# Twinklebear/tray_rust

Hardware: NVIDIA H100
Metric: Mrays/s (primary+secondary) (higher is better)
Workload: dtype f32

## Files before the change

### tray_rust_b200/csrc/trb_api.cu

```cuda
#include <chrono>
#include <dlfcn.h>
#include <nccl.h>
#include <cstdio>
#include <cstdlib>
#include <memory>
#include <thread>
#include <tuple>
#include <cub/device/device_radix_sort.cuh>
#include "trb_host.h"
#include "trb_kernels.cuh"
#include "trb_bvh_build.cuh"
#include "trb_denoise.cuh"

using namespace trbh;

namespace {

thread_local std::string g_error;
unsigned long long g_launches = 0;
trb_status fail(trb_status s, const std::string& msg) { g_error = msg; return s; }

#define CU(call)                                                                                                   \
    do {                                                                                                           \
        cudaError_t e_ = (call);                                                                                   \
// ... 119 lines not shown
        q.q[2 * k + 1] = make_float4(in[node].bmax[0], in[node].bmax[1], in[node].bmax[2], 0.f);
    };
    for (size_t qi = 0; qi < order.size(); ++qi) {
        const uint32_t p = order[qi];
        trb::DQuad& q = out[qi];
        uint32_t axes[2] = {0, 0};
        int h = 0;
        for (uint32_t c : {p + 1, in[p].a}) {
            bool split = false;
            if (!is_leaf(c)) { const uint32_t g0 = c + 1, g1 = in[c].a; split = inside(g0, c) && inside(g1, c); }
            if (split) { slot(q, 2 * h, c + 1, false); slot(q, 2 * h + 1, in[c].a, false); axes[h] = in[c].b & 3u; }
            else { slot(q, 2 * h, c, false); slot(q, 2 * h + 1, 0, true); }
            ++h;
        }
        q.q[1].w = bits_f((in[p].b & 3u) | axes[0] << 2 | axes[1] << 4);
    }
    root_ref = trb::REF_INTERIOR | quad_of[0];
    return ok;
}

}

namespace {
struct Tuning {
    int refill = 8;
    unsigned trace_grid = 0;
    uint32_t sched = 6;
    int quads = 0;
    int exact_box = 0;
    int wide_leaf = 0;
    int pipe = 36;
    int film_v2 = 1;
    int sort = 0;
    int sort_bits = 5;
    int sort_min_round = 1;
    int shade_anim_occ = 4;
    int frame_device = 1;
    int anim_table = 2;
    int shade_split = -1;
    int shade_sort = 1;
    int shade_kind = 1;
    uint64_t pass_paths = 1ull << 24;
    int build_device = 1;
    long long tlas_min = -1;
    int frame_time = 0;
    int tlas_small = 8;
};
constexpr uint32_t kTlasLevelMin = 256;
int env_int(const char* name, int dflt) { const char* v = getenv(name); return v ? (int)strtol(v, nullptr, 0) : dflt; }
void tuning_from_env(Tuning& t) {
    t.refill = env_int("TRB_REFILL", t.refill); t.trace_grid = (unsigned)env_int("TRB_TRACE_GRID", (int)t.trace_grid);
    t.sched = (uint32_t)env_int("TRB_TRACE_SCHED", (int)t.sched); t.quads = env_int("TRB_TRACE_QUADS", t.quads); t.pipe = env_int("TRB_TRACE_PIPE", t.pipe);
    t.wide_leaf = env_int("TRB_TRACE_WIDE_LEAF", t.wide_leaf);
    t.film_v2 = env_int("TRB_FILM_V2", t.film_v2); t.sort = env_int("TRB_SORT", t.sort); t.sort_bits = env_int("TRB_SORT_BITS", t.sort_bits);
    t.sort_min_round = env_int("TRB_SORT_MIN_ROUND", t.sort_min_round); t.shade_split = env_int("TRB_SHADE_SPLIT", t.shade_split); t.anim_table = env_int("TRB_ANIM_TABLE", t.anim_table); t.frame_device = env_int("TRB_FRAME_DEVICE", t.frame_device);
    if (getenv("TRB_PASS_PATHS")) t.pass_paths = strtoull(getenv("TRB_PASS_PATHS"), nullptr, 0);
    t.build_device = env_int("TRB_BUILD_DEVICE", t.build_device);
    t.tlas_min = env_int("TRB_FRAME_TLAS_MIN", (int)t.tlas_min); t.frame_time = env_int("TRB_FRAME_TIME", t.frame_time);
    t.tlas_small = std::max(4, env_int("TRB_FRAME_TLAS_SMALL", t.tlas_small));
}

}

struct BlockList {
    uint32_t key[5];
    std::vector<uint32_t> host;
    uint2* dev = nullptr;
};

struct trb_scene {
    int device = 0;
    int sm_count = 0;
    Tuning tune;
    trb_film film{};
    trb_integrator integrator{};
    std::vector<trb_camera> cameras;
// ... 322 lines not shown
    }
    s->wf_capacity = cap;
    return TRB_OK;
}

void launch_anim_table(trb_scene* s, trb::WfState& wf, size_t n_paths, bool adapt, cudaStream_t st) {
    if (!(s->ds.has_anim && wf.xf_tab && s->tune.anim_table)) { wf.xf_tab = nullptr; return; }
    const size_t items = n_paths * wf.n_anim;
    const uint32_t nu = s->ds.n_uniq_splines;
    if (s->tune.anim_table >= 2 && nu > 0 && nu <= 256) {
        const uint32_t per_iter = std::max(1u, std::min(32u, 128u / nu));
        const size_t smem = (size_t)per_iter * nu * 32 * sizeof(float);
        const unsigned grid = (unsigned)std::min<size_t>((n_paths + per_iter - 1) / per_iter, (size_t)s->sm_count * 16);
        if (adapt) trb::k_wf_anim_table2<true><<<grid, 128, smem, st>>>(s->ds, wf, per_iter);
        else trb::k_wf_anim_table2<<<grid, 128, smem, st>>>(s->ds, wf, per_iter);
    } else {
        const unsigned grid = (unsigned)std::min<size_t>((items + 127) / 128, (size_t)s->sm_count * 16);
        if (adapt) trb::k_wf_anim_table<true><<<grid, 128, 0, st>>>(s->ds, wf);
        else trb::k_wf_anim_table<<<grid, 128, 0, st>>>(s->ds, wf);
    }
    g_launches++;
}

void launch_query_trace(trb_scene* s, const trb::RenderParams& rp, const trb::WfState& wf, uint32_t tflags, bool stats, const uint32_t* q_sorted,
                        cudaStream_t st) {
    const Tuning& tu = s->tune;
    const bool anim = s->ds.has_anim != 0;
    const unsigned resident = stats ? 4u : (anim ? 8u : 9u);
    const unsigned tgrid = (unsigned)s->sm_count * (tu.trace_grid ? tu.trace_grid : 2u * resident);
    const uint32_t sched = std::max(1u, tu.sched);
    if (s->wide_leaf) {
        if (anim) {
            if (stats) trb::k_wf_trace<true, 4, 16, true, true, false, 225><<<tgrid, 128, 0, st>>>(s->ds, rp, wf, 0, tflags, tu.refill, sched, q_sorted);
            else trb::k_wf_trace<false, 8, 12, true, true, false, 225><<<tgrid, 128, 0, st>>>(s->ds, rp, wf, 0, tflags, tu.refill, sched, q_sorted);
        } else if (stats) trb::k_wf_trace<true, 4, 16, false, true, false, 225><<<tgrid, 128, 0, st>>>(s->ds, rp, wf, 0, tflags, tu.refill, sched, q_sorted);
        else trb::k_wf_trace<false, 9, 12, false, true, false, 225><<<tgrid, 128, 0, st>>>(s->ds, rp, wf, 0, tflags, tu.refill, sched, q_sorted);
    } else if (anim) {
        if (stats) trb::k_wf_trace<true, 4, 16, true, true, false, 97><<<tgrid, 128, 0, st>>>(s->ds, rp, wf, 0, tflags, tu.refill, sched, q_sorted);
        else trb::k_wf_trace<false, 8, 12, true, true, false, 97><<<tgrid, 128, 0, st>>>(s->ds, rp, wf, 0, tflags, tu.refill, sched, q_sorted);
    } else if (stats) trb::k_wf_trace<true, 4, 16, false, true, false, 97><<<tgrid, 128, 0, st>>>(s->ds, rp, wf, 0, tflags, tu.refill, sched, q_sorted);
    else trb::k_wf_trace<false, 9, 12, false, true, false, 97><<<tgrid, 128, 0, st>>>(s->ds, rp, wf, 0, tflags, tu.refill, sched, q_sorted);
}

template <int MODE>
void launch_shade(trb_scene* s, const trb::RenderParams& rp, const trb::WfState& wf, uint32_t round, cudaStream_t st) {
    const Tuning& tu = s->tune;
    const bool anim = s->ds.has_anim != 0;
    const unsigned shade_grid = (unsigned)s->sm_count * 4;
    const bool split_auto = s->mixed_materials || (tu.shade_sort && tu.shade_kind && s->material_kinds == (1u << TRB_MAT_MATTE));
    if (tu.shade_split > 0 || (tu.shade_split < 0 && split_auto)) {
        const uint32_t all = 0xffu, own = (tu.shade_sort && tu.shade_kind) ? (s->material_kinds & (1u << TRB_MAT_MATTE)) : 0u;
        const uint32_t rest = tu.shade_sort ? (s->material_kinds & ~own) : all;
        if (anim) {
            trb::k_wf_shade_a<MODE, true, 3><<<shade_grid, 128, 0, st>>>(s->ds, rp, wf, round);
            if (own) trb::k_wf_shade_b<true, 4, TRB_MAT_MATTE><<<shade_grid, 128, 0, st>>>(s->ds, rp, wf, round, own);
            if (rest) trb::k_wf_shade_b<true, 3><<<shade_grid, 128, 0, st>>>(s->ds, rp, wf, round, rest);
            if (own) trb::k_wf_shade_c<MODE, true, 6, TRB_MAT_MATTE><<<(unsigned)s->sm_count * 6, 128, 0, st>>>(s->ds, rp, wf, round, own);
            if (rest) trb::k_wf_shade_c<MODE, true, 4><<<shade_grid, 128, 0, st>>>(s->ds, rp, wf, round, rest);
        } else {
            const unsigned ga = (unsigned)s->sm_count * 6, gb = (unsigned)s->sm_count * 5, gc = (unsigned)s->sm_count * 6;
            trb::k_wf_shade_a<MODE, false, 6><<<ga, 128, 0, st>>>(s->ds, rp, wf, round);
            if (own) trb::k_wf_shade_b<false, 5, TRB_MAT_MATTE><<<gb, 128, 0, st>>>(s->ds, rp, wf, round, own);
            if (rest) trb::k_wf_shade_b<false, 5><<<gb, 128, 0, st>>>(s->ds, rp, wf, round, rest);
            if (own) trb::k_wf_shade_c<MODE, false, 6, TRB_MAT_MATTE><<<gc, 128, 0, st>>>(s->ds, rp, wf, round, own);
// ... 2 lines not shown
        g_launches += 4;
        return;
    }
    if (anim) {
        if constexpr (MODE == 1) trb::k_wf_shade<1, true, 3><<<shade_grid, 128, 0, st>>>(s->ds, rp, wf, round);
        else if constexpr (MODE == 2) trb::k_wf_shade<2, true, 4><<<shade_grid, 128, 0, st>>>(s->ds, rp, wf, round);
        else if (tu.shade_anim_occ >= 4) trb::k_wf_shade<0, true, 4><<<shade_grid, 128, 0, st>>>(s->ds, rp, wf, round);
        else trb::k_wf_shade<0, true, 3><<<shade_grid, 128, 0, st>>>(s->ds, rp, wf, round);
    } else trb::k_wf_shade<MODE, false, 4><<<shade_grid, 128, 0, st>>>(s->ds, rp, wf, round);
    g_launches += 2;
}

trb_status wavefront_rounds(trb_scene* s, const trb::RenderParams& rp, const trb::WfState& wf, uint32_t flags, int mode, cudaStream_t st,
                            const AovRequest* aov = nullptr) {
    const Tuning& tu = s->tune;
    const bool stats = (flags & TRB_RENDER_STATS) != 0, anim = s->ds.has_anim != 0;
    const uint32_t rounds = s->integrator.max_depth + 2;
    const int refill = tu.refill;
    const unsigned resident = (flags & TRB_RENDER_STATS) ? 4u : (tu.pipe == 0 || tu.pipe == 1 || tu.pipe == 33 ? 7u : (tu.pipe == 34 || tu.pipe == 35 || s->ds.has_anim ? 8u : 9u));
    const unsigned tgrid = (unsigned)s->sm_count * (tu.trace_grid ? tu.trace_grid : 2u * resident);
    const uint32_t sched = tu.sched;
    const bool quads = tu.quads != 0;
    const uint32_t tflags = flags | (tu.exact_box ? trb::WF_TRACE_FORCE_EXACT_BOX : 0u);
    if (s->wide_leaf && (sched == 0 || quads || tu.pipe == 0 || tu.pipe == 1 || (tu.pipe >= 33 && tu.pipe <= 35) || tu.pipe == 37))
        return fail(TRB_UNSUPPORTED, "trace.quads, trace.sched 0 and the experimental trace.pipe variants do not read wide mesh leaves (trace.wide_leaf)");
    if (quads && s->quads_dropped) return fail(TRB_UNSUPPORTED, "trace.quads reads DQuad records, which a mesh updated by trb_scene_update_mesh does not have");
    for (uint32_t round = 0; round < rounds; ++round) {
        const uint32_t* q_sorted = nullptr;
        if (tu.sort && (int)round >= tu.sort_min_round) {
            const uint32_t bits = (uint32_t)std::min(trb::WF_SORT_MAX_BITS, std::max(1, tu.sort_bits));
            const unsigned sgrid = (unsigned)s->sm_count * 8;
            trb::k_wf_sort_count<<<sgrid, 256, 0, st>>>(wf, round, bits, tu.sort == 2 ? 1u : 0u);
            trb::k_wf_sort_scan<<<1, 1024, 0, st>>>(wf, 3u * (8u << (3u * bits)));
            trb::k_wf_sort_scatter<<<sgrid, 256, 0, st>>>(wf, round);
            g_launches += 3;
            q_sorted = wf.q_sorted;
        }
        std::pair<cudaEvent_t, cudaEvent_t> ev{nullptr, nullptr};
        if (flags & TRB_RENDER_TIME_TRACE) {
            if (!s->event_pool.empty()) { ev = s->event_pool.back(); s->event_pool.pop_back(); }
            else { CU(cudaEventCreate(&ev.first)); CU(cudaEventCreate(&ev.second)); }
            CU(cudaEventRecord(ev.first, st));
        }
#define TRB_TRACE_LAUNCH(ST, MB, SS, AN, PH, QD, PIPE) trb::k_wf_trace<ST, MB, SS, AN, PH, QD, PIPE><<<tgrid, 128, 0, st>>>(s->ds, rp, wf, round, tflags, refill, sched, q_sorted)
        const bool v2 = tu.pipe != 0;
        if (mode == 2 && round == 0) launch_query_trace(s, rp, wf, tflags, stats, q_sorted, st);
        else if (s->wide_leaf) {
            if (anim) { if (stats) TRB_TRACE_LAUNCH(true, 4, 16, true, true, false, 161); else TRB_TRACE_LAUNCH(false, 8, 12, true, true, false, 161); }
            else if (stats) TRB_TRACE_LAUNCH(true, 4, 16, false, true, false, 161);
            else TRB_TRACE_LAUNCH(false, 9, 12, false, true, false, 161);
        } else if (anim) {
            if (stats) { if (v2) TRB_TRACE_LAUNCH(true, 4, 16, true, true, false, 33); else TRB_TRACE_LAUNCH(true, 4, 16, true, true, false, 0); }
            else if (!v2) TRB_TRACE_LAUNCH(false, 7, 16, true, true, false, 0);
            else if (tu.pipe == 33) TRB_TRACE_LAUNCH(false, 7, 16, true, true, false, 33);
            else if (tu.pipe == 37) TRB_TRACE_LAUNCH(false, 9, 12, true, true, false, 33);
            else TRB_TRACE_LAUNCH(false, 8, 12, true, true, false, 33);
        } else if (stats) {
            if (sched == 0) TRB_TRACE_LAUNCH(true, 4, 16, false, false, false, 0);
            else if (v2) TRB_TRACE_LAUNCH(true, 4, 16, false, true, false, 33); else TRB_TRACE_LAUNCH(true, 4, 16, false, true, false, 0);
        } else if (sched == 0) TRB_TRACE_LAUNCH(false, 7, 16, false, false, false, 0);
        else if (quads) TRB_TRACE_LAUNCH(false, 7, 16, false, true, true, 0);
        else switch (tu.pipe) {
            case 0: TRB_TRACE_LAUNCH(false, 7, 16, false, true, false, 0); break;
            case 1: TRB_TRACE_LAUNCH(false, 7, 16, false, true, false, 1); break;
            case 33: TRB_TRACE_LAUNCH(false, 7, 16, false, true, false, 33); break;
            case 34: TRB_TRACE_LAUNCH(false, 8, 16, false, true, false, 33); break;
            case 35: TRB_TRACE_LAUNCH(false, 8, 12, false, true, false, 33); break;
            case 37: TRB_TRACE_LAUNCH(false, 9, 8, false, true, false, 33); break;
            default: TRB_TRACE_LAUNCH(false, 9, 12, false, true, false, 33); break;
        }
#undef TRB_TRACE_LAUNCH
        if (ev.first) { CU(cudaEventRecord(ev.second, st)); s->trace_events.push_back(ev); }
        if (aov && round == 0) {
            const unsigned agrid = (unsigned)std::min<size_t>((wf.n_paths + 127) / 128, (size_t)s->sm_count * 16);
            float4* lo = mode == 1 ? reinterpret_cast<float4*>(aov->samples) : s->d_aov;
            float4* hi = mode == 1 ? lo + 1 : s->d_aov + s->aov_capacity;
            const uint32_t step = mode == 1 ? 2u : 1u;
            if (anim) trb::k_wf_aov<true><<<agrid, 128, 0, st>>>(s->ds, wf, lo, hi, step);
            else trb::k_wf_aov<false><<<agrid, 128, 0, st>>>(s->ds, wf, lo, hi, step);
            g_launches++;
        }
        if (mode == 0) launch_shade<0>(s, rp, wf, round, st);
        else if (mode == 1) launch_shade<1>(s, rp, wf, round, st);
        else launch_shade<2>(s, rp, wf, round, st);
    }
    CU(cudaGetLastError());
    return TRB_OK;
}

trb_status launch_wavefront(trb_scene* s, const trb::RenderParams& rp, uint32_t flags, int mode, cudaStream_t st, const AovRequest* aov = nullptr) {
    const size_t n_paths = (size_t)rp.n_blocks * 64 * rp.sample_count;
    if (n_paths > s->wf_capacity || n_paths >= (1ull << 30)) return fail(TRB_INVALID_ARG, "pass larger than the wavefront state");
    const Tuning& tu = s->tune;
// ... 1375 lines not shown
uint32_t trb_abi_version(void) { return TRB_ABI_VERSION; }
unsigned long long trb_launch_count(void) { return g_launches; }

trb_status trb_scene_set_option(trb_scene* s, const char* name, long long value) {
    if (!s || !name) return fail(TRB_INVALID_ARG, "null argument");
    Tuning& t = s->tune;
    const std::string k(name);
    if (k == "trace.refill") t.refill = (int)value;
    else if (k == "trace.occupancy" || k == "trace.smem_stack") {}
    else if (k == "trace.grid") t.trace_grid = (unsigned)std::max<long long>(0, value);
    else if (k == "trace.sched") t.sched = (uint32_t)value;
    else if (k == "trace.quads" || k == "frame.device") {
        int& field = k == "trace.quads" ? t.quads : t.frame_device;
        const bool changed = (field != 0) != (value != 0);
        field = (int)value;
        if (changed && s->frame_set) return trb_scene_update_frame(s, s->last_frame, s->last_start, s->last_end);
    }
    else if (k == "frame.tlas_min") {
        const bool changed = t.tlas_min != value;
        t.tlas_min = value;
        if (changed && s->frame_set) return trb_scene_update_frame(s, s->last_frame, s->last_start, s->last_end);
    }
    else if (k == "trace.pipe") t.pipe = (int)value;
    else if (k == "trace.exact_box") t.exact_box = (int)value;
    else if (k == "trace.wide_leaf") {
        t.wide_leaf = (int)value;
        const bool wide = s->needs_wide || value != 0;
        if (wide != s->wide_leaf) { CU(cudaSetDevice(s->device)); return upload_mesh_nodes(s, wide); }
    }
    else if (k == "film.v2") t.film_v2 = (int)value;
    else if (k == "sort.mode") t.sort = (int)value;
    else if (k == "sort.bits") t.sort_bits = (int)std::min<long long>(6, std::max<long long>(1, value));
    else if (k == "sort.min_round") t.sort_min_round = (int)value;
    else if (k == "shade.split") t.shade_split = (int)value;
    else if (k == "shade.sort") t.shade_sort = (int)value;
    else if (k == "shade.kind") t.shade_kind = (int)value;
    else if (k == "anim.table") t.anim_table = (int)value;
    else if (k == "shade.anim_occupancy") t.shade_anim_occ = (int)value;
    else if (k == "pass.paths") { if (value < 64) return fail(TRB_INVALID_ARG, "pass.paths must be >= 64"); t.pass_paths = (uint64_t)value; }
    else return fail(TRB_INVALID_ARG, "unknown option: " + k);
    return TRB_OK;
}

trb_status trb_scene_check_error(trb_scene* s) {
    if (!s) return fail(TRB_INVALID_ARG, "null scene");
    CU(cudaSetDevice(s->device));
// ... 2183 lines not shown
```

### tray_rust_b200/csrc/trb_kernels.cuh

```cuda
#pragma once
#include "trb_device.h"
#include "trb_detmath.cuh"
#include "trb_anim.h"
#include "trb_adaptive.h"
#include "../../include/trb.h"

namespace trb {

struct f3 { float x, y, z; };
TRB_HD __forceinline__ f3 mk(float x, float y, float z) { f3 r; r.x = x; r.y = y; r.z = z; return r; }
__device__ __forceinline__ f3 splat(float v) { return mk(v, v, v); }
__device__ __forceinline__ f3 operator+(f3 a, f3 b) { return mk(a.x + b.x, a.y + b.y, a.z + b.z); }
__device__ __forceinline__ f3 operator-(f3 a, f3 b) { return mk(a.x - b.x, a.y - b.y, a.z - b.z); }
__device__ __forceinline__ f3 operator*(f3 a, f3 b) { return mk(a.x * b.x, a.y * b.y, a.z * b.z); }
__device__ __forceinline__ float ieee_div(float a, float b) { return a / b; }
__device__ __forceinline__ float ieee_sqrt(float a) { return sqrtf(a); }
__device__ __forceinline__ f3 operator/(f3 a, f3 b) { return mk(ieee_div(a.x, b.x), ieee_div(a.y, b.y), ieee_div(a.z, b.z)); }
__device__ __forceinline__ f3 operator*(f3 a, float s) { return mk(a.x * s, a.y * s, a.z * s); }
__device__ __forceinline__ f3 operator*(float s, f3 a) { return mk(s * a.x, s * a.y, s * a.z); }
__device__ __forceinline__ f3 operator/(f3 a, float s) { return mk(ieee_div(a.x, s), ieee_div(a.y, s), ieee_div(a.z, s)); }
__device__ __forceinline__ f3 operator-(f3 a) { return mk(-a.x, -a.y, -a.z); }
__device__ __forceinline__ float dot3(f3 a, f3 b) { return a.x * b.x + a.y * b.y + a.z * b.z; }
__device__ __forceinline__ f3 cross3(f3 a, f3 b) { return mk(a.y * b.z - a.z * b.y, a.z * b.x - a.x * b.z, a.x * b.y - a.y * b.x); }
__device__ __forceinline__ float len2(f3 a) { return a.x * a.x + a.y * a.y + a.z * a.z; }
// ... 322 lines not shown
                const float p0 = __ldg(&in.p0), p1 = __ldg(&in.p1);
                float tt = t.tmax;
                bool h;
                if (shape == TRB_SHAPE_SPHERE) h = sphere_t(p0, lo_, ld_, t.tmin, tt);
                else if (shape == TRB_SHAPE_DISK) h = disk_t(p0, p1, lo_, ld_, t.tmin, tt);
                else h = rect_t(p0, p1, lo_, ld_, t.tmin, tt);
                if (h) {
                    t.tmax = tt;
                    t.h_inst = ii; t.h_prim = 0; t.h_b1 = 0.0f; t.h_b2 = 0.0f;
                    t.found = true;
                    if (t.any_hit) t.sp = 0;
                }
            }
        }
        if (!enter) next = trace_pop(t, stack);
    }
    t.cur = next;
}

constexpr uint32_t ST_POP = 0xfffffffcu;
constexpr uint32_t WF_TRACE_FORCE_EXACT_BOX = 0x40000000u;
constexpr int WF_BURST = 3;
__device__ __forceinline__ bool trace_is_node(uint32_t cur) { return (cur & REF_TAG) == REF_INTERIOR || cur == ST_POP; }
template <bool STATS, bool QUADS, class Stack>
__device__ __forceinline__ void step_nodes(TraceState& t, const Stack& stack, Cnt& cnt, int* err) {
    uint32_t cur = t.cur;
    if (QUADS && cur != ST_POP && t.quad) {
        const float4* __restrict__ rec = reinterpret_cast<const DQuad*>(t.pairs)[cur].q;
        float4 q0, q1, q2, q3, q4, q5, q6, q7;
        ldg256(rec, q0, q1); ldg256(rec + 2, q2, q3); ldg256(rec + 4, q4, q5); ldg256(rec + 6, q6, q7);
        QuadOut qo;
        quad_visit(q0, q1, q2, q3, q4, q5, q6, q7, t.o, t.inv, (t.neg & 1u) != 0, (t.neg & 2u) != 0, (t.neg & 4u) != 0, t.tmin, t.tmax, qo);
        cur = qo.next == QUAD_EMPTY ? ST_POP : qo.next;
        if (qo.p2) {
            if (t.sp >= STACK_DEPTH - 6) { *err = 1; t.sp = 0; cur = ST_DONE; }
            else {
                if (qo.p0) stack.put(t.sp++, qo.e0);
                if (qo.p1) stack.put(t.sp++, qo.e1);
                stack.put(t.sp++, qo.e2);
            }
        } else if (qo.p0 || qo.p1) {
            if (t.sp >= STACK_DEPTH - 6) { *err = 1; t.sp = 0; cur = ST_DONE; }
            else {
                if (qo.p0) stack.put(t.sp++, qo.e0);
                if (qo.p1) stack.put(t.sp++, qo.e1);
            }
// ... 42 lines not shown
    return (h & 4u) ? (u * 2.0f - 1.0f) * 30.0f : (u * 2.0f - 1.0f);
}
__global__ void k_selftest_box(uint32_t n, uint32_t seed, unsigned long long* out) {
    const uint32_t i = blockIdx.x * blockDim.x + threadIdx.x;
    if (i >= n) return;
    uint32_t h = rng_absorb(rng_seed(seed), i);
    float v[14];
    for (int k = 0; k < 14; ++k) { h = mix32(h + 0x9e3779b9u); v[k] = selftest_value(h); }
    const float4 lo = make_float4(fminf(v[0], v[3]), fminf(v[1], v[4]), fminf(v[2], v[5]), 0.0f), hi = make_float4(fmaxf(v[0], v[3]), fmaxf(v[1], v[4]), fmaxf(v[2], v[5]), 0.0f);
    f3 o = mk(v[6], v[7], v[8]);
    if ((h & 0x30u) == 0) o.x = lo.x;
    if ((h & 0xc0u) == 0) o.y = hi.y;
    const f3 d = mk(v[9], v[10], v[11]);
    const f3 inv = mk(1.0f / d.x, 1.0f / d.y, 1.0f / d.z);
    const float tmin = (h & 0x100u) ? 0.0f : 0.001f, tmax = (h & 0x200u) ? finf() : fabsf(v[12]) * 40.0f;
    const bool nx = d.x < 0.0f, ny = d.y < 0.0f, nz = d.z < 0.0f;
    if (!(finite3(o) && finite3(d) && finite3(inv))) { atomicAdd(&out[3], 1ull); return; }
    float ta = 0.0f, tb = 0.0f;
    const bool a = box_hit(lo, hi, o, inv, nx, ny, nz, tmin, tmax, ta), b = box_hit_finite(lo, hi, o, inv, nx, ny, nz, tmin, tmax, tb);
    atomicAdd(&out[0], 1ull);
    if (a) atomicAdd(&out[1], 1ull);
    if (a != b || (a && !(ta == tb))) atomicAdd(&out[2], 1ull);
}
template <bool STATS, bool FAST, class Stack>
__device__ __forceinline__ void step_nodes2(TraceState& t, const Stack& stack, Cnt& cnt, int* err) {
    uint32_t cur = t.cur;
    if (cur != ST_POP) {
        const DPair* __restrict__ rec = t.pairs + cur;
        float4 l_lo, l_hi, r_lo, r_hi;
        ldg256(&rec->l_lo, l_lo, l_hi);
        ldg256(&rec->r_lo, r_lo, r_hi);
        if (STATS) cnt.node += 2;
        const uint32_t axis = __float_as_uint(r_lo.w);
        const bool neg = ((t.neg >> axis) & 1u) != 0;
        const uint32_t ref_l = __float_as_uint(l_lo.w), ref_r = __float_as_uint(l_hi.w);
        const bool nx = (t.neg & 1u) != 0, ny = (t.neg & 2u) != 0, nz = (t.neg & 4u) != 0;
        float tl, tr;
        bool hl, hr;
        if (FAST && !t.exact_box) {
            hl = box_hit_finite(l_lo, l_hi, t.o, t.inv, nx, ny, nz, t.tmin, t.tmax, tl);
            hr = box_hit_finite(r_lo, r_hi, t.o, t.inv, nx, ny, nz, t.tmin, t.tmax, tr);
        } else {
            hl = box_hit(l_lo, l_hi, t.o, t.inv, nx, ny, nz, t.tmin, t.tmax, tl);
            hr = box_hit(r_lo, r_hi, t.o, t.inv, nx, ny, nz, t.tmin, t.tmax, tr);
        }
        const bool both = hl && hr;
        cur = both ? (neg ? ref_r : ref_l) : (hl ? ref_l : (hr ? ref_r : ST_POP));
        if (both) {
            if (t.sp >= STACK_DEPTH - 6) { *err = 1; t.sp = 0; cur = ST_DONE; }
            else stack.put(t.sp++, ((unsigned long long)__float_as_uint(neg ? tl : tr) << 32) | (neg ? ref_l : ref_r));
        }
    }
#pragma unroll
    for (int k = 0; k < 2; ++k) {
// ... 23 lines not shown
        float4 v0, q0, q1, qpad;
        ldg256(&tri->v0, v0, q0);
        ldg256(&tri->e1, q1, qpad);
        if (WIDE) next = __float_as_uint(q0.w) == TRI_LEAF_END ? ST_POP : cur + 1;
        if (STATS) cnt.tri++;
        const f3 e0 = mk(q0.x, q0.y, q0.z), e1 = mk(q1.x, q1.y, q1.z);
        const f3 s0 = cross3(t.d, e1);
        const float dd = dot3(s0, e0);
        const float div = 1.0f / dd;
        const f3 dv = t.o - mk(v0.x, v0.y, v0.z);
        const float b1 = dot3(dv, s0) * div;
        const f3 s1 = cross3(dv, e0);
        const float b2 = dot3(t.d, s1) * div;
        const float tt = dot3(e1, s1) * div;
        const bool ok = dd != 0.0f && !(b1 < 0.0f || b1 > 1.0f) && !(b2 < 0.0f || b1 + b2 > 1.0f) && !(tt < t.tmin || tt > t.tmax);
        if (ok) {
            t.tmax = tt;
            accept_hit<HOME>(t, home, t.level_inst, __float_as_uint(v0.w), b1, b2);
            if (t.any_hit) { t.sp = 0; next = ST_DONE; }
        }
    }
    t.cur = next;
}
template <bool STATS, bool ANIM, bool HOME = false, class Stack>
__device__ __forceinline__ void step_other(const DScene& sc, TraceState& t, const Stack& stack, Cnt& cnt, const RayHome* home = nullptr) {
    uint32_t cur = t.cur;
    uint32_t next = ST_POP;
    bool inst_now = false;
    if ((cur & REF_TAG) == REF_LEAF) {
        const uint32_t a = cur & 0x01ffffffu, n = (cur >> 25) & 31u;
        if (HOME) {
            for (uint32_t k = a + n; k-- > a + 1;) stack.put(t.sp++, ST_INSTANCE | k);
            cur = ST_INSTANCE | a; inst_now = n != 0;
        } else
            for (uint32_t k = a + n; k-- > a;) stack.put(t.sp++, ST_INSTANCE | k);
    } else if (cur == ST_ROOT) {
        const DBvh* bvh = t.bvh;
        if (HOME) bvh = t.level_inst == TRB_MISS ? sc.tlas : &sc.meshes[__ldg(&sc.instances[t.level_inst].mesh)].bvh;
        const float4 lo = __ldg(&bvh->root_lo), hi = __ldg(&bvh->root_hi);
        if (STATS) cnt.node++;
        float te;
        if (box_hit(lo, hi, t.o, t.inv, (t.neg & 1u) != 0, (t.neg & 2u) != 0, (t.neg & 4u) != 0, t.tmin, t.tmax, te)) next = __float_as_uint(t.quad ? hi.w : lo.w);
    } else if (cur == ST_RETURN) {
        if (HOME) {
            const float4 o4 = __ldcs(home->org), d4 = __ldcs(home->dir);
            t.o = mk(o4.x, o4.y, o4.z); t.d = mk(d4.x, d4.y, d4.z);
            t.inv = mk(1.0f / t.d.x, 1.0f / t.d.y, 1.0f / t.d.z);
        } else { t.o = t.wo; t.d = t.wd; t.inv = t.winv; }
        t.neg = neg_mask(t.d);
        trace_level(t, sc.tlas, sc.tlas_pairs, sc.tlas_quads);
        t.level_inst = TRB_MISS;
    } else inst_now = true;
    if (inst_now) {
        const uint32_t ii = __ldg(&sc.tlas_order[cur & ~REF_TAG]);
        const DInstance& in = sc.instances[ii];
        if (STATS) cnt.inst++;
        const uint32_t kind = __ldg(&in.kind), shape = __ldg(&in.shape);
        if (kind != TRB_INST_EMITTER_POINT) {
            float m[16];
            instance_inv<ANIM>(sc, in, t.time, m, t.xf_row);
            const f3 lo_ = xf_point(m, HOME ? t.o : t.wo), ld_ = xf_vector(m, HOME ? t.d : t.wd);
            if (shape == TRB_SHAPE_MESH) {
                const DMesh& me = sc.meshes[__ldg(&in.mesh)];
                const f3 inv_ = mk(1.0f / ld_.x, 1.0f / ld_.y, 1.0f / ld_.z);
                const uint32_t neg_ = neg_mask(ld_);
                bool enter = true;
                next = ST_ROOT;
                if (HOME) {
                    const float4 lo = __ldg(&me.bvh.root_lo), hi = __ldg(&me.bvh.root_hi);
                    if (STATS) cnt.node++;
                    float te;
                    enter = box_hit(lo, hi, lo_, inv_, (neg_ & 1u) != 0, (neg_ & 2u) != 0, (neg_ & 4u) != 0, t.tmin, t.tmax, te);
                    next = enter ? __float_as_uint(lo.w) : ST_POP;
                }
                if (enter) {
                    t.o = lo_; t.d = ld_; t.inv = inv_; t.neg = neg_;
                    trace_level(t, &me.bvh, me.bvh.pairs, me.bvh.quads);
                    t.tris = me.tris; t.level_inst = ii;
                    stack.put(t.sp++, ST_RETURN);
                }
            } else {
                const float p0 = __ldg(&in.p0), p1 = __ldg(&in.p1);
                float tt = t.tmax;
                bool h;
                if (shape == TRB_SHAPE_SPHERE) h = sphere_t(p0, lo_, ld_, t.tmin, tt);
                else if (shape == TRB_SHAPE_DISK) h = disk_t(p0, p1, lo_, ld_, t.tmin, tt);
                else h = rect_t(p0, p1, lo_, ld_, t.tmin, tt);
                if (h) {
                    t.tmax = tt;
                    accept_hit<HOME>(t, home, ii, 0u, 0.0f, 0.0f);
                    if (t.any_hit) { t.sp = 0; next = ST_DONE; }
                }
            }
        }
    }
    t.cur = next;
// ... 1206 lines not shown
        const PixelStreams ps = pixel_streams(rp.seed, id.pixel);
        float sx, sy, tm;
        sample_position(rp, ps, id, sx, sy, tm);
        Ray ray;
        const float time = camera_ray<ANIM>(sc, sx, sy, tm, ray);
        wf.org[p] = make_float4(ray.o.x, ray.o.y, ray.o.z, __uint_as_float(0u));
        wf.cont[p] = make_float4(ray.d.x, ray.d.y, ray.d.z, finf());
        wf.thr[p] = make_float4(1.0f, 1.0f, 1.0f, time);
        wf.illum[p] = make_float4(0.0f, 0.0f, 0.0f, 0.0f);
        wf.q_cont[p] = p;
    }
    if (blockIdx.x == 0 && threadIdx.x == 0) {
        wf.counters[WF_N_ACTIVE] = n; wf.counters[WF_N_CONT] = n;
        if (rp.stats) { atomicAdd(&rp.stats->camera_samples, (unsigned long long)n); }
    }
    if (wf.bounds && blockIdx.x == 0 && threadIdx.x < 64) {
        uint32_t* b = wf.bounds + threadIdx.x * 8;
        b[0] = b[1] = b[2] = b[3] = 0xffffffffu; b[4] = b[5] = b[6] = b[7] = 0u;
    }
}

template <bool STATS, int MINB, int SMEM_STACK, bool ANIM, bool PHASED, bool QUADS, int PIPE = 0>
__global__ void __launch_bounds__(128, MINB) k_wf_trace(const __grid_constant__ DScene sc, const __grid_constant__ RenderParams rp, const __grid_constant__ WfState wf,
                                                         uint32_t round, uint32_t flags, int WF_REFILL_IDLE, uint32_t sched, const uint32_t* __restrict__ q_sorted) {
    constexpr bool HOME = PHASED && (PIPE & 32) != 0;
    constexpr bool QUERY = (PIPE & 64) != 0;
    constexpr bool WIDE = (PIPE & 128) != 0;
    uint32_t* cnt_r = wf.counters + round * WF_CNT;
    const uint32_t n_cont = cnt_r[WF_N_CONT], n_shadow = cnt_r[WF_N_SHADOW], n_mis = cnt_r[WF_N_MIS];
    const uint32_t total = n_cont + n_shadow + n_mis;
    const bool shadow_any = (flags & 4u) == 0;
    const int lane = threadIdx.x & 31;
    const unsigned lt_mask = (1u << lane) - 1u;
    Cnt cnt = {0, 0, 0};
    TraceState t;
    __shared__ unsigned long long s_stack[SMEM_STACK * 128];
    unsigned long long stack_lo[STACK_DEPTH - SMEM_STACK];
    const HybridStack<SMEM_STACK> stack{s_stack + threadIdx.x, stack_lo};
    t.cur = ST_DONE;
    bool have = false, exhausted = false;
    uint32_t p = 0;
    int type = 0;
    for (;;) {
        if (HOME && have && t.cur == ST_DONE) {
            if (type == 0) {
                __stcs(&wf.cont[p].w, t.tmax);
                if (!t.found) __stcs(&wf.hit[p], make_uint4(TRB_MISS, 0u, 0u, 0u));
            } else if (type == 1) __stcs(&wf.shadow[p].w, __uint_as_float(t.found ? 1u : 0u));
            else {
                __stcs(&wf.mis[p].w, t.tmax);
                if (!t.found) __stcs(&wf.a[p].w, __uint_as_float(TRB_MISS));
            }
            have = false;
        } else if (have && t.cur == ST_DONE) {
            if (type == 0) {
                __stcs(&wf.cont[p], make_float4(t.wd.x, t.wd.y, t.wd.z, t.tmax));
                __stcs(&wf.hit[p], make_uint4(t.found ? t.h_inst : TRB_MISS, t.h_prim, __float_as_uint(t.h_b1), __float_as_uint(t.h_b2)));
            } else if (type == 1) {
                __stcs(&wf.shadow[p], make_float4(t.wd.x, t.wd.y, t.wd.z, __uint_as_float(t.found ? 1u : 0u)));
            } else {
                __stcs(&wf.mis[p], make_float4(t.wd.x, t.wd.y, t.wd.z, t.tmax));
// ... 9 lines not shown
            uint32_t base = 0;
            if (lane == leader) base = atomicAdd(&cnt_r[WF_TRACE_HEAD], (uint32_t)__popc(idle));
            base = __shfl_sync(0xffffffffu, base, leader);
            if (base >= total) exhausted = true;
            else if (!have) {
                const uint32_t i = base + __popc(idle & lt_mask);
                if (i < total) {
                    if (q_sorted) { const uint32_t e = __ldg(&q_sorted[i]); type = (int)(e >> 30); p = e & WF_PATH_MASK; }
                    else if (i < n_cont) { type = 0; p = wf.q_cont[i]; }
                    else if (i < n_cont + n_shadow) { type = 1; p = wf.q_shadow[i - n_cont]; }
                    else { type = 2; p = wf.q_mis[i - n_cont - n_shadow]; }
                    const float4 o4 = __ldcs(&wf.org[p]);
                    const float4 d4 = __ldcs(type == 0 ? &wf.cont[p] : (type == 1 ? &wf.shadow[p] : &wf.mis[p]));
                    Ray ray; ray.o = mk(o4.x, o4.y, o4.z); ray.d = mk(d4.x, d4.y, d4.z);
                    ray.tmin = QUERY ? o4.w : ((type == 0 && round == 0) ? 0.0f : 0.001f);
                    ray.tmax = QUERY ? d4.w : (type == 1 ? 0.999f : finf());
                    trace_init(sc, t, ray, type == 1 && shadow_any, ANIM ? __ldg(&wf.thr[p].w) : 0.0f, QUADS && PHASED, (flags & WF_TRACE_FORCE_EXACT_BOX) != 0);
                    t.xf_row = wf_xf_row<ANIM>(wf, p);
                    if (PHASED) { stack.put(0, (unsigned long long)ST_DONE); t.sp = 1; }
                    if (HOME) {
                        const float4 lo = __ldg(&sc.tlas->root_lo), hi = __ldg(&sc.tlas->root_hi);
                        if (STATS) cnt.node++;
                        float te;
                        t.cur = box_hit(lo, hi, t.o, t.inv, (t.neg & 1u) != 0, (t.neg & 2u) != 0, (t.neg & 4u) != 0, t.tmin, t.tmax, te) ? __float_as_uint(lo.w) : ST_POP;
                    }
                    have = true;
                }
            }
        }
        const unsigned busy0 = __ballot_sync(0xffffffffu, have);
        if (busy0 == 0) { if (exhausted) break; else continue; }
        if (PHASED) {
            const int thr_o = (int)(sched & 255u);
            for (;;) {
#pragma unroll
                for (int k = 0; k < WF_BURST; ++k)
                    if (trace_is_node(t.cur)) {
                        if (PIPE != 0 && !QUADS) step_nodes2<STATS, (PIPE & 1) != 0>(t, stack, cnt, rp.error_flag);
                        else step_nodes<STATS, QUADS>(t, stack, cnt, rp.error_flag);
                    }
                const bool is_a = trace_is_node(t.cur), is_o = !is_a && t.cur != ST_DONE;
                const unsigned m_a = __ballot_sync(0xffffffffu, is_a), m_o = __ballot_sync(0xffffffffu, is_o);
                if ((m_a | m_o) == 0) break;
                if (!exhausted && 32 - __popc(m_a | m_o) >= WF_REFILL_IDLE) break;
                if (m_o != 0 && (m_a == 0 || __popc(m_o) >= thr_o)) {
                    if (is_o) {
                        const RayHome home{&wf.org[p], type == 0 ? &wf.cont[p] : (type == 1 ? &wf.shadow[p] : &wf.mis[p]), &wf.hit[p], &wf.a[p].w, type};
                        if ((t.cur & REF_TAG) == REF_LEAF && t.level_inst != TRB_MISS) step_triangle<STATS, HOME, WIDE>(t, cnt, &home);
                        else step_other<STATS, ANIM, HOME>(sc, t, stack, cnt, &home);
                    }
                }
            }
        } else {
            for (;;) {
                if (have && t.cur != ST_DONE) trace_step<STATS, ANIM, WIDE>(sc, t, stack, cnt, rp.error_flag);
                const unsigned running = __ballot_sync(0xffffffffu, have && t.cur != ST_DONE);
                if (running == 0) break;
                if (!exhausted && 32 - __popc(running) >= WF_REFILL_IDLE) break;
            }
        }
    }
    if (rp.stats) {
        if (STATS) {
            unsigned long long v[3] = {cnt.node, cnt.tri, cnt.inst};
            for (int k = 0; k < 3; ++k) {
                unsigned long long x = v[k];
                for (int o = 16; o > 0; o >>= 1) x += __shfl_xor_sync(0xffffffffu, x, o);
                if (lane == 0 && x) atomicAdd(&rp.stats->node_tests + k, x);
            }
        }
        if (blockIdx.x == 0 && threadIdx.x == 0) {
            atomicAdd(round == 0 ? &rp.stats->rays_primary : &rp.stats->rays_continuation, (unsigned long long)n_cont);
// ... 1136 lines not shown
```

Measured before the change: 779.5.

## Add optional shared-memory BVH top-node cache and raise refill threshold

```diff
diff --git a/tray_rust_b200/csrc/trb_api.cu b/tray_rust_b200/csrc/trb_api.cu
--- a/tray_rust_b200/csrc/trb_api.cu
+++ b/tray_rust_b200/csrc/trb_api.cu
@@ -165,14 +165,16 @@
 }
 
 namespace {
+constexpr uint32_t NODE_CACHE_DEFAULT = 0, NODE_CACHE_MAX = 480;
 struct Tuning {
-    int refill = 8;
+    int refill = 16;
     unsigned trace_grid = 0;
     uint32_t sched = 6;
     int quads = 0;
     int exact_box = 0;
     int wide_leaf = 0;
     int pipe = 36;
+    uint32_t node_cache = NODE_CACHE_DEFAULT;
     int film_v2 = 1;
     int sort = 0;
     int sort_bits = 5;
@@ -195,6 +197,7 @@
     t.refill = env_int("TRB_REFILL", t.refill); t.trace_grid = (unsigned)env_int("TRB_TRACE_GRID", (int)t.trace_grid);
     t.sched = (uint32_t)env_int("TRB_TRACE_SCHED", (int)t.sched); t.quads = env_int("TRB_TRACE_QUADS", t.quads); t.pipe = env_int("TRB_TRACE_PIPE", t.pipe);
     t.wide_leaf = env_int("TRB_TRACE_WIDE_LEAF", t.wide_leaf);
+    t.node_cache = (uint32_t)std::min<int>((int)NODE_CACHE_MAX, std::max(0, env_int("TRB_TRACE_NODE_CACHE", (int)t.node_cache)));
     t.film_v2 = env_int("TRB_FILM_V2", t.film_v2); t.sort = env_int("TRB_SORT", t.sort); t.sort_bits = env_int("TRB_SORT_BITS", t.sort_bits);
     t.sort_min_round = env_int("TRB_SORT_MIN_ROUND", t.sort_min_round); t.shade_split = env_int("TRB_SHADE_SPLIT", t.shade_split); t.anim_table = env_int("TRB_ANIM_TABLE", t.anim_table); t.frame_device = env_int("TRB_FRAME_DEVICE", t.frame_device);
     if (getenv("TRB_PASS_PATHS")) t.pass_paths = strtoull(getenv("TRB_PASS_PATHS"), nullptr, 0);
@@ -563,6 +566,20 @@
     g_launches++;
 }
 
+struct NodeCacheArgs { uint32_t records, mesh; };
+NodeCacheArgs node_cache_args(const trb_scene* s) {
+    NodeCacheArgs a{s->tune.node_cache, TRB_MISS};
+    if (a.records == 0 || s->tlas_n_nodes >= trb::CACHE_BASE) return {0u, TRB_MISS};
+    uint32_t best = 0;
+    for (const trb_instance& in : s->instances) {
+        if (in.shape != TRB_SHAPE_MESH || in.mesh >= s->dmeshes.size()) continue;
+        const trb::DMesh& m = s->dmeshes[in.mesh];
+        if (m.n_nodes >= trb::CACHE_BASE) return {0u, TRB_MISS};
+        if (a.mesh == TRB_MISS || m.n_tris > best) { a.mesh = in.mesh; best = m.n_tris; }
+    }
+    return a;
+}
+
 void launch_query_trace(trb_scene* s, const trb::RenderParams& rp, const trb::WfState& wf, uint32_t tflags, bool stats, const uint32_t* q_sorted,
                         cudaStream_t st) {
     const Tuning& tu = s->tune;
@@ -570,17 +587,22 @@
     const unsigned resident = stats ? 4u : (anim ? 8u : 9u);
     const unsigned tgrid = (unsigned)s->sm_count * (tu.trace_grid ? tu.trace_grid : 2u * resident);
     const uint32_t sched = std::max(1u, tu.sched);
+    const NodeCacheArgs nc = node_cache_args(s);
+#define TRB_QUERY_LAUNCH(ST, MB, AN, PIPE) \
+    if (nc.records) trb::k_wf_trace<ST, MB, ST ? 16 : 12, AN, true, false, PIPE | 256><<<tgrid, 128, nc.records * sizeof(trb::DPair), st>>>(s->ds, rp, wf, 0, tflags, tu.refill, sched, q_sorted, nc.records, nc.mesh); \
+    else trb::k_wf_trace<ST, MB, ST ? 16 : 12, AN, true, false, PIPE><<<tgrid, 128, 0, st>>>(s->ds, rp, wf, 0, tflags, tu.refill, sched, q_sorted, 0u, TRB_MISS)
     if (s->wide_leaf) {
         if (anim) {
-            if (stats) trb::k_wf_trace<true, 4, 16, true, true, false, 225><<<tgrid, 128, 0, st>>>(s->ds, rp, wf, 0, tflags, tu.refill, sched, q_sorted);
-            else trb::k_wf_trace<false, 8, 12, true, true, false, 225><<<tgrid, 128, 0, st>>>(s->ds, rp, wf, 0, tflags, tu.refill, sched, q_sorted);
-        } else if (stats) trb::k_wf_trace<true, 4, 16, false, true, false, 225><<<tgrid, 128, 0, st>>>(s->ds, rp, wf, 0, tflags, tu.refill, sched, q_sorted);
-        else trb::k_wf_trace<false, 9, 12, false, true, false, 225><<<tgrid, 128, 0, st>>>(s->ds, rp, wf, 0, tflags, tu.refill, sched, q_sorted);
+            if (stats) { TRB_QUERY_LAUNCH(true, 4, true, 225); }
+            else { TRB_QUERY_LAUNCH(false, 8, true, 225); }
+        } else if (stats) { TRB_QUERY_LAUNCH(true, 4, false, 225); }
+        else { TRB_QUERY_LAUNCH(false, 9, false, 225); }
     } else if (anim) {
-        if (stats) trb::k_wf_trace<true, 4, 16, true, true, false, 97><<<tgrid, 128, 0, st>>>(s->ds, rp, wf, 0, tflags, tu.refill, sched, q_sorted);
-        else trb::k_wf_trace<false, 8, 12, true, true, false, 97><<<tgrid, 128, 0, st>>>(s->ds, rp, wf, 0, tflags, tu.refill, sched, q_sorted);
-    } else if (stats) trb::k_wf_trace<true, 4, 16, false, true, false, 97><<<tgrid, 128, 0, st>>>(s->ds, rp, wf, 0, tflags, tu.refill, sched, q_sorted);
-    else trb::k_wf_trace<false, 9, 12, false, true, false, 97><<<tgrid, 128, 0, st>>>(s->ds, rp, wf, 0, tflags, tu.refill, sched, q_sorted);
+        if (stats) { TRB_QUERY_LAUNCH(true, 4, true, 97); }
+        else { TRB_QUERY_LAUNCH(false, 8, true, 97); }
+    } else if (stats) { TRB_QUERY_LAUNCH(true, 4, false, 97); }
+    else { TRB_QUERY_LAUNCH(false, 9, false, 97); }
+#undef TRB_QUERY_LAUNCH
 }
 
 template <int MODE>
@@ -629,6 +651,7 @@
     const uint32_t sched = tu.sched;
     const bool quads = tu.quads != 0;
     const uint32_t tflags = flags | (tu.exact_box ? trb::WF_TRACE_FORCE_EXACT_BOX : 0u);
+    const NodeCacheArgs nc = node_cache_args(s);
     if (s->wide_leaf && (sched == 0 || quads || tu.pipe == 0 || tu.pipe == 1 || (tu.pipe >= 33 && tu.pipe <= 35) || tu.pipe == 37))
         return fail(TRB_UNSUPPORTED, "trace.quads, trace.sched 0 and the experimental trace.pipe variants do not read wide mesh leaves (trace.wide_leaf)");
     if (quads && s->quads_dropped) return fail(TRB_UNSUPPORTED, "trace.quads reads DQuad records, which a mesh updated by trb_scene_update_mesh does not have");
@@ -649,22 +672,25 @@
             else { CU(cudaEventCreate(&ev.first)); CU(cudaEventCreate(&ev.second)); }
             CU(cudaEventRecord(ev.first, st));
         }
-#define TRB_TRACE_LAUNCH(ST, MB, SS, AN, PH, QD, PIPE) trb::k_wf_trace<ST, MB, SS, AN, PH, QD, PIPE><<<tgrid, 128, 0, st>>>(s->ds, rp, wf, round, tflags, refill, sched, q_sorted)
+#define TRB_TRACE_LAUNCH(ST, MB, SS, AN, PH, QD, PIPE) trb::k_wf_trace<ST, MB, SS, AN, PH, QD, PIPE><<<tgrid, 128, 0, st>>>(s->ds, rp, wf, round, tflags, refill, sched, q_sorted, 0u, TRB_MISS)
+#define TRB_TRACE_LAUNCH_NC(ST, MB, SS, AN, PIPE) \
+        if (nc.records) trb::k_wf_trace<ST, MB, SS, AN, true, false, PIPE | 256><<<tgrid, 128, nc.records * sizeof(trb::DPair), st>>>(s->ds, rp, wf, round, tflags, refill, sched, q_sorted, nc.records, nc.mesh); \
+        else TRB_TRACE_LAUNCH(ST, MB, SS, AN, true, false, PIPE)
         const bool v2 = tu.pipe != 0;
         if (mode == 2 && round == 0) launch_query_trace(s, rp, wf, tflags, stats, q_sorted, st);
         else if (s->wide_leaf) {
-            if (anim) { if (stats) TRB_TRACE_LAUNCH(true, 4, 16, true, true, false, 161); else TRB_TRACE_LAUNCH(false, 8, 12, true, true, false, 161); }
-            else if (stats) TRB_TRACE_LAUNCH(true, 4, 16, false, true, false, 161);
-            else TRB_TRACE_LAUNCH(false, 9, 12, false, true, false, 161);
+            if (anim) { if (stats) { TRB_TRACE_LAUNCH_NC(true, 4, 16, true, 161); } else { TRB_TRACE_LAUNCH_NC(false, 8, 12, true, 161); } }
+            else if (stats) { TRB_TRACE_LAUNCH_NC(true, 4, 16, false, 161); }
+            else { TRB_TRACE_LAUNCH_NC(false, 9, 12, false, 161); }
         } else if (anim) {
-            if (stats) { if (v2) TRB_TRACE_LAUNCH(true, 4, 16, true, true, false, 33); else TRB_TRACE_LAUNCH(true, 4, 16, true, true, false, 0); }
+            if (stats) { if (v2) { TRB_TRACE_LAUNCH_NC(true, 4, 16, true, 33); } else TRB_TRACE_LAUNCH(true, 4, 16, true, true, false, 0); }
             else if (!v2) TRB_TRACE_LAUNCH(false, 7, 16, true, true, false, 0);
             else if (tu.pipe == 33) TRB_TRACE_LAUNCH(false, 7, 16, true, true, false, 33);
             else if (tu.pipe == 37) TRB_TRACE_LAUNCH(false, 9, 12, true, true, false, 33);
-            else TRB_TRACE_LAUNCH(false, 8, 12, true, true, false, 33);
+            else { TRB_TRACE_LAUNCH_NC(false, 8, 12, true, 33); }
         } else if (stats) {
             if (sched == 0) TRB_TRACE_LAUNCH(true, 4, 16, false, false, false, 0);
-            else if (v2) TRB_TRACE_LAUNCH(true, 4, 16, false, true, false, 33); else TRB_TRACE_LAUNCH(true, 4, 16, false, true, false, 0);
+            else if (v2) { TRB_TRACE_LAUNCH_NC(true, 4, 16, false, 33); } else TRB_TRACE_LAUNCH(true, 4, 16, false, true, false, 0);
         } else if (sched == 0) TRB_TRACE_LAUNCH(false, 7, 16, false, false, false, 0);
         else if (quads) TRB_TRACE_LAUNCH(false, 7, 16, false, true, true, 0);
         else switch (tu.pipe) {
@@ -674,8 +700,9 @@
             case 34: TRB_TRACE_LAUNCH(false, 8, 16, false, true, false, 33); break;
             case 35: TRB_TRACE_LAUNCH(false, 8, 12, false, true, false, 33); break;
             case 37: TRB_TRACE_LAUNCH(false, 9, 8, false, true, false, 33); break;
-            default: TRB_TRACE_LAUNCH(false, 9, 12, false, true, false, 33); break;
+            default: TRB_TRACE_LAUNCH_NC(false, 9, 12, false, 33); break;
         }
+#undef TRB_TRACE_LAUNCH_NC
 #undef TRB_TRACE_LAUNCH
         if (ev.first) { CU(cudaEventRecord(ev.second, st)); s->trace_events.push_back(ev); }
         if (aov && round == 0) {
@@ -2097,6 +2124,10 @@
         if (changed && s->frame_set) return trb_scene_update_frame(s, s->last_frame, s->last_start, s->last_end);
     }
     else if (k == "trace.pipe") t.pipe = (int)value;
+    else if (k == "trace.node_cache") {
+        if (value < 0 || value > (long long)NODE_CACHE_MAX) return fail(TRB_INVALID_ARG, "trace.node_cache must be 0..480 records");
+        t.node_cache = (uint32_t)value;
+    }
     else if (k == "trace.exact_box") t.exact_box = (int)value;
     else if (k == "trace.wide_leaf") {
         t.wide_leaf = (int)value;
diff --git a/tray_rust_b200/csrc/trb_kernels.cuh b/tray_rust_b200/csrc/trb_kernels.cuh
--- a/tray_rust_b200/csrc/trb_kernels.cuh
+++ b/tray_rust_b200/csrc/trb_kernels.cuh
@@ -368,6 +368,43 @@
 constexpr uint32_t WF_TRACE_FORCE_EXACT_BOX = 0x40000000u;
 constexpr int WF_BURST = 3;
 __device__ __forceinline__ bool trace_is_node(uint32_t cur) { return (cur & REF_TAG) == REF_INTERIOR || cur == ST_POP; }
+
+constexpr uint32_t CACHE_BASE = (1u << 30) - (1u << 16);
+__device__ __noinline__ void node_cache_stage(const DScene& sc, float4* nc, uint32_t cap, uint32_t mesh, uint32_t* roots, uint32_t* s_n) {
+    uint32_t begin = 0;
+    for (int tree = 0; tree < 2; ++tree) {
+        if (tree == 1 && mesh == TRB_MISS) break;
+        const DBvh* bvh = tree == 0 ? sc.tlas : &sc.meshes[mesh].bvh;
+        const DPair* pairs = bvh->pairs;
+        if (threadIdx.x == 0) {
+            const uint32_t root = __float_as_uint(__ldg(&bvh->root_lo.w));
+            roots[tree] = root;
+            if ((root & REF_TAG) == REF_INTERIOR && begin < cap) { nc[begin].w = __uint_as_float(root); roots[tree] = CACHE_BASE + begin; }
+            *s_n = roots[tree] >= CACHE_BASE ? begin + 1 : begin;
+        }
+        __syncthreads();
+        uint32_t end = roots[tree] >= CACHE_BASE ? begin + 1 : begin;
+        while (begin < end) {
+            for (uint32_t s = begin + threadIdx.x; s < end; s += blockDim.x) {
+                const DPair* rec = pairs + __float_as_uint(nc[s].w);
+                float4 l_lo, l_hi, r_lo, r_hi;
+                ldg256(&rec->l_lo, l_lo, l_hi);
+                ldg256(&rec->r_lo, r_lo, r_hi);
+                uint32_t ref[2] = {__float_as_uint(l_lo.w), __float_as_uint(l_hi.w)};
+                for (int c = 0; c < 2; ++c)
+                    if ((ref[c] & REF_TAG) == REF_INTERIOR) {
+                        const uint32_t k = atomicAdd(s_n, 1u);
+                        if (k < cap) { nc[k].w = __uint_as_float(ref[c]); ref[c] = CACHE_BASE + k; }
+                    }
+                l_lo.w = __uint_as_float(ref[0]); l_hi.w = __uint_as_float(ref[1]);
+                nc[s] = l_lo; nc[cap + s] = l_hi; nc[2 * cap + s] = r_lo; nc[3 * cap + s] = r_hi;
+            }
+            __syncthreads();
+            begin = end; end = min(*s_n, cap);
+            __syncthreads();
+        }
+    }
+}
 template <bool STATS, bool QUADS, class Stack>
 __device__ __forceinline__ void step_nodes(TraceState& t, const Stack& stack, Cnt& cnt, int* err) {
     uint32_t cur = t.cur;
@@ -456,14 +493,19 @@
     if (a) atomicAdd(&out[1], 1ull);
     if (a != b || (a && !(ta == tb))) atomicAdd(&out[2], 1ull);
 }
-template <bool STATS, bool FAST, class Stack>
-__device__ __forceinline__ void step_nodes2(TraceState& t, const Stack& stack, Cnt& cnt, int* err) {
+template <bool STATS, bool FAST, bool NC = false, class Stack>
+__device__ __forceinline__ void step_nodes2(TraceState& t, const Stack& stack, Cnt& cnt, int* err, const float4* nc = nullptr, uint32_t nc_stride = 0) {
     uint32_t cur = t.cur;
     if (cur != ST_POP) {
-        const DPair* __restrict__ rec = t.pairs + cur;
         float4 l_lo, l_hi, r_lo, r_hi;
-        ldg256(&rec->l_lo, l_lo, l_hi);
-        ldg256(&rec->r_lo, r_lo, r_hi);
+        if (NC && cur >= CACHE_BASE) {
+            const float4* s = nc + (cur - CACHE_BASE);
+            l_lo = s[0]; l_hi = s[nc_stride]; r_lo = s[2 * nc_stride]; r_hi = s[3 * nc_stride];
+        } else {
+            const DPair* __restrict__ rec = t.pairs + cur;
+            ldg256(&rec->l_lo, l_lo, l_hi);
+            ldg256(&rec->r_lo, r_lo, r_hi);
+        }
         if (STATS) cnt.node += 2;
         const uint32_t axis = __float_as_uint(r_lo.w);
         const bool neg = ((t.neg >> axis) & 1u) != 0;
@@ -533,8 +575,9 @@
     }
     t.cur = next;
 }
-template <bool STATS, bool ANIM, bool HOME = false, class Stack>
-__device__ __forceinline__ void step_other(const DScene& sc, TraceState& t, const Stack& stack, Cnt& cnt, const RayHome* home = nullptr) {
+template <bool STATS, bool ANIM, bool HOME = false, bool NC = false, class Stack>
+__device__ __forceinline__ void step_other(const DScene& sc, TraceState& t, const Stack& stack, Cnt& cnt, const RayHome* home = nullptr,
+                                           const uint32_t* nc_roots = nullptr, uint32_t nc_mesh = 0) {
     uint32_t cur = t.cur;
     uint32_t next = ST_POP;
     bool inst_now = false;
@@ -572,7 +615,8 @@
             instance_inv<ANIM>(sc, in, t.time, m, t.xf_row);
             const f3 lo_ = xf_point(m, HOME ? t.o : t.wo), ld_ = xf_vector(m, HOME ? t.d : t.wd);
             if (shape == TRB_SHAPE_MESH) {
-                const DMesh& me = sc.meshes[__ldg(&in.mesh)];
+                const uint32_t mi = __ldg(&in.mesh);
+                const DMesh& me = sc.meshes[mi];
                 const f3 inv_ = mk(1.0f / ld_.x, 1.0f / ld_.y, 1.0f / ld_.z);
                 const uint32_t neg_ = neg_mask(ld_);
                 bool enter = true;
@@ -582,7 +626,7 @@
                     if (STATS) cnt.node++;
                     float te;
                     enter = box_hit(lo, hi, lo_, inv_, (neg_ & 1u) != 0, (neg_ & 2u) != 0, (neg_ & 4u) != 0, t.tmin, t.tmax, te);
-                    next = enter ? __float_as_uint(lo.w) : ST_POP;
+                    next = enter ? ((NC && mi == nc_mesh) ? nc_roots[1] : __float_as_uint(lo.w)) : ST_POP;
                 }
                 if (enter) {
                     t.o = lo_; t.d = ld_; t.inv = inv_; t.neg = neg_;
@@ -1835,10 +1879,12 @@
 
 template <bool STATS, int MINB, int SMEM_STACK, bool ANIM, bool PHASED, bool QUADS, int PIPE = 0>
 __global__ void __launch_bounds__(128, MINB) k_wf_trace(const __grid_constant__ DScene sc, const __grid_constant__ RenderParams rp, const __grid_constant__ WfState wf,
-                                                         uint32_t round, uint32_t flags, int WF_REFILL_IDLE, uint32_t sched, const uint32_t* __restrict__ q_sorted) {
+                                                         uint32_t round, uint32_t flags, int WF_REFILL_IDLE, uint32_t sched, const uint32_t* __restrict__ q_sorted,
+                                                         uint32_t nc_records, uint32_t nc_mesh) {
     constexpr bool HOME = PHASED && (PIPE & 32) != 0;
     constexpr bool QUERY = (PIPE & 64) != 0;
     constexpr bool WIDE = (PIPE & 128) != 0;
+    constexpr bool NC = HOME && (PIPE & 256) != 0;
     uint32_t* cnt_r = wf.counters + round * WF_CNT;
     const uint32_t n_cont = cnt_r[WF_N_CONT], n_shadow = cnt_r[WF_N_SHADOW], n_mis = cnt_r[WF_N_MIS];
     const uint32_t total = n_cont + n_shadow + n_mis;
@@ -1850,6 +1896,9 @@
     __shared__ unsigned long long s_stack[SMEM_STACK * 128];
     unsigned long long stack_lo[STACK_DEPTH - SMEM_STACK];
     const HybridStack<SMEM_STACK> stack{s_stack + threadIdx.x, stack_lo};
+    extern __shared__ float4 s_nc[];
+    __shared__ uint32_t s_nc_roots[2], s_nc_n;
+    if (NC) node_cache_stage(sc, s_nc, nc_records, nc_mesh, s_nc_roots, &s_nc_n);
     t.cur = ST_DONE;
     bool have = false, exhausted = false;
     uint32_t p = 0;
@@ -1905,7 +1954,7 @@
                         const float4 lo = __ldg(&sc.tlas->root_lo), hi = __ldg(&sc.tlas->root_hi);
                         if (STATS) cnt.node++;
                         float te;
-                        t.cur = box_hit(lo, hi, t.o, t.inv, (t.neg & 1u) != 0, (t.neg & 2u) != 0, (t.neg & 4u) != 0, t.tmin, t.tmax, te) ? __float_as_uint(lo.w) : ST_POP;
+                        t.cur = box_hit(lo, hi, t.o, t.inv, (t.neg & 1u) != 0, (t.neg & 2u) != 0, (t.neg & 4u) != 0, t.tmin, t.tmax, te) ? (NC ? s_nc_roots[0] : __float_as_uint(lo.w)) : ST_POP;
                     }
                     have = true;
                 }
@@ -1919,7 +1968,7 @@
 #pragma unroll
                 for (int k = 0; k < WF_BURST; ++k)
                     if (trace_is_node(t.cur)) {
-                        if (PIPE != 0 && !QUADS) step_nodes2<STATS, (PIPE & 1) != 0>(t, stack, cnt, rp.error_flag);
+                        if (PIPE != 0 && !QUADS) step_nodes2<STATS, (PIPE & 1) != 0, NC>(t, stack, cnt, rp.error_flag, s_nc, nc_records);
                         else step_nodes<STATS, QUADS>(t, stack, cnt, rp.error_flag);
                     }
                 const bool is_a = trace_is_node(t.cur), is_o = !is_a && t.cur != ST_DONE;
@@ -1930,7 +1979,7 @@
                     if (is_o) {
                         const RayHome home{&wf.org[p], type == 0 ? &wf.cont[p] : (type == 1 ? &wf.shadow[p] : &wf.mis[p]), &wf.hit[p], &wf.a[p].w, type};
                         if ((t.cur & REF_TAG) == REF_LEAF && t.level_inst != TRB_MISS) step_triangle<STATS, HOME, WIDE>(t, cnt, &home);
-                        else step_other<STATS, ANIM, HOME>(sc, t, stack, cnt, &home);
+                        else step_other<STATS, ANIM, HOME, NC>(sc, t, stack, cnt, &home, s_nc_roots, nc_mesh);
                     }
                 }
             }
```

After: 796.3, median of 6. 1.02x the previous value.
